# ChaoqinRobotics/LINS---LiDAR-inertial-SLAM

Measured on NVIDIA H100. Metric: ESKF iterations/sec, higher is better.
Workload: dtype f64 (f32 association)

## Files before the change

lins---lidar-inertial-slam_b200/csrc/cuda/lins_assoc_az.cuh:

```cuda
#pragma once
#include "lins_kernels.cuh"

namespace lins_dev {

struct AzIndex {
  const float4* pts;
  const aztab_t* bstart;
  const int (*elev)[2];
  int nb, nrings, T;
};
__device__ __forceinline__ int float_key(float f) { const int i = __float_as_int(f); return i >= 0 ? i : i ^ 0x7fffffff; }
__device__ __forceinline__ float key_float(int k) { return __int_as_float(k >= 0 ? k : k ^ 0x7fffffff); }
__device__ __forceinline__ float slope_of(float x, float y, float z) {
  return __fdiv_rn(z, sqrtf(__fadd_rn(__fmul_rn(x, x), __fmul_rn(y, y))));
}
__device__ __forceinline__ float ring_lower_bound(const AzIndex& ix, int r, float zq, float rq) {
  const float lo = key_float(ix.elev[r][0]), hi = key_float(ix.elev[r][1]);
  const float a = __fmaf_rn(lo, rq, -zq), b = __fmaf_rn(-hi, rq, zq);
  const float m = a > b ? lo : hi;
  const float bound = fmaxf(a, b) * rsqrtf(__fmaf_rn(m, m, 1.f)) * 0.998f - 1.0e-4f;
  return hi - lo < 1.0e30f ? bound : -1.f;
}

__device__ __forceinline__ int az_bin(float x, float y, int nb) {
  const float a = atan2f(y, x);
  int b = (int)floorf((a + kPiF) * ((float)nb * (0.5f / kPiF)));
  return min(max(b, 0), nb - 1);
}
__device__ __forceinline__ int az_bins_for(int nrings, int tab) {
  int p2 = 1;
  while (p2 < nrings) p2 <<= 1;
  return tab / p2;
}

__device__ __forceinline__ int cnt16_add1(unsigned* cnt, int b) {
  const int sh = (b & 1) * 16;
  return (int)((atomicAdd(&cnt[b >> 1], 1u << sh) >> sh) & 0xffffu);
}
template <int TAB>
__device__ void az_build(const float4* __restrict__ src, int T, float4* dst, aztab_t* table, unsigned* cnt, int* scan_tmp, int nb, int (*elev)[2]) {
  unsigned short* cnt16 = reinterpret_cast<unsigned short*>(cnt);
  for (int w = threadIdx.x; w <= TAB / 2; w += kThreads) cnt[w] = 0u;
  for (int r = threadIdx.x; r < kMaxRing; r += kThreads) { elev[r][0] = float_key(3.0e38f); elev[r][1] = float_key(-3.0e38f); }
  __syncthreads();
  for (int j = threadIdx.x; j < T; j += kThreads) {
    const float4 t = __ldg(&src[j]);
    cnt16_add1(cnt, (int)t.w * nb + az_bin(t.x, t.y, nb));
    const float e = slope_of(t.x, t.y, t.z);
    if (fabsf(e) < 1.0e30f) { const int k = float_key(e); atomicMin(&elev[(int)t.w][0], k); atomicMax(&elev[(int)t.w][1], k); }
    else { atomicMin(&elev[(int)t.w][0], float_key(-3.0e38f)); atomicMax(&elev[(int)t.w][1], float_key(3.0e38f)); }
  }
  __syncthreads();
  constexpr int PER = TAB / kThreads;
  static_assert(PER >= 1 && PER * kThreads == TAB, "table size must be a multiple of the block size");
  int loc[PER];
  int sum = 0;
#pragma unroll
  for (int k = 0; k < PER; ++k) { loc[k] = cnt16[threadIdx.x * PER + k]; sum += loc[k]; }
  scan_tmp[threadIdx.x] = sum;
  __syncthreads();
  if (threadIdx.x < 32) {
    constexpr int PW = kThreads / 32;
    int part[PW];
    int s = 0;
#pragma unroll
    for (int k = 0; k < PW; ++k) { part[k] = scan_tmp[threadIdx.x * PW + k]; s += part[k]; }
    int incl = s;
#pragma unroll
    for (int m = 1; m < 32; m <<= 1) { const int o = __shfl_up_sync(0xffffffffu, incl, m); if ((int)threadIdx.x >= m) incl += o; }
    int run = incl - s;
#pragma unroll
    for (int k = 0; k < PW; ++k) { const int v = part[k]; scan_tmp[threadIdx.x * PW + k] = run; run += v; }
    if (threadIdx.x == 31) table[TAB] = (aztab_t)incl;
  }
  __syncthreads();
  {
    int run = scan_tmp[threadIdx.x];
#pragma unroll
    for (int k = 0; k < PER; ++k) { cnt16[threadIdx.x * PER + k] = (unsigned short)run; table[threadIdx.x * PER + k] = (aztab_t)run; run += loc[k]; }
  }
  __syncthreads();
  for (int j = threadIdx.x; j < T; j += kThreads) {
    const float4 t = __ldg(&src[j]);
    const int pos = cnt16_add1(cnt, (int)t.w * nb + az_bin(t.x, t.y, nb));
    dst[pos] = make_float4(t.x, t.y, t.z, __int_as_float(((int)t.w << 24) | j));
  }
  __syncthreads();
}

__device__ __forceinline__ float az_halfwidth(float U, float rho) {
  const float r = sqrtf(U) * 1.002f + 1.0e-5f;
  if (!(r < rho)) return 4.0f;
  return asinf(r / rho) + 1.0e-5f;
}
__device__ __forceinline__ void az_window(int nb, float aq, float th, int& blo, int& nbins) {
  const float inv_binw = (float)nb * (0.5f / kPiF);
  nbins = (int)(2.0f * th * inv_binw) + 3;
  if (!(th < kPiF) || nbins >= nb) { blo = 0; nbins = nb; return; }
  int b = (int)floorf((aq - th + kPiF) * inv_binw) - 1;
  b %= nb;
  if (b < 0) b += nb;
  blo = b;
}

__device__ __forceinline__ int slot_index(float w) { return __float_as_int(w) & 0x00ffffff; }
__device__ __forceinline__ int slot_ring(float w) { return (int)((unsigned)__float_as_int(w) >> 24); }
__device__ __forceinline__ int pack_window(int blo, int nbins) { return (blo << 16) | nbins; }
constexpr float kCertMargin = 0.1f;
__device__ __forceinline__ float widen(float U) { const float r = sqrtf(U) + kCertMargin; return r * r; }
__device__ __forceinline__ float rejected_slack(unsigned best_bits, float Bout, float gate) {
  const float db = best_bits >= 0x7f800000u ? Bout : fminf(sqrtf(__uint_as_float(best_bits)), Bout);
  return db - gate * 1.00001f;
}

__device__ __forceinline__ void az_polar(const float4 s, float4& qa) {
  qa.x = atan2f(s.y, s.x);
  qa.y = sqrtf(__fadd_rn(__fmul_rn(s.x, s.x), __fmul_rn(s.y, s.y)));
}
__device__ __forceinline__ int az_nn_window(const AzIndex& ix, float U1, float4& qa) {
  const float Uw = widen(U1);
  int blo, nbins;
  az_window(ix.nb, qa.x, az_halfwidth(Uw, qa.y), blo, nbins);
  qa.w = nbins >= ix.nb ? 3.0e38f : sqrtf(Uw);
  return pack_window(blo, nbins);
}
__device__ __forceinline__ float az_seed_bound(const AzIndex& ix, const float4 s, int seed_slot, float U1) {
  if (seed_slot >= 0 && seed_slot < ix.T) {
    const float4 t = ix.pts[seed_slot];
    const float d = sqdist_f32(s.x, s.y, s.z, t.x, t.y, t.z);
    if (d < U1) U1 = d;
  }
  return U1;
}
__device__ __forceinline__ int az_bin_of_angle(float a, int nb) {
  const int b = (int)floorf((a + kPiF) * ((float)nb * (0.5f / kPiF)));
  return min(max(b, 0), nb - 1);
}
__device__ __forceinline__ float az_bucket_bound(const AzIndex& ix, const float4 s, float az, int ring_guess, float U1) {
  const int bq = az_bin_of_angle(az, ix.nb);
  const int r0 = min(max(ring_guess, 0), ix.nrings - 1);
#pragma unroll 1
  for (int k = 0; k < 3; ++k) {
    const int r = k == 0 ? r0 : (k == 1 ? r0 - 1 : r0 + 1);
    if (k == 1 && U1 < 1.0f) break;
    if (r < 0 || r >= ix.nrings) continue;
    const int base = r * ix.nb;
    int p = ix.bstart[base + max(bq - 1, 0)];
    const int pe = min((int)ix.bstart[base + min(bq + 2, ix.nb)], p + 4);
    for (; p < pe; ++p) U1 = az_seed_bound(ix, s, p, U1);
  }
  return U1;
}
__device__ __forceinline__ int az_prepare_nn(const AzIndex& ix, const float4 s, float nearf, int seed_slot, int ring_guess, float4& qa) {
  qa = make_float4(0.f, 0.f, -1.f, 0.f);
  if (!(s.x == s.x && s.y == s.y && s.z == s.z) || ix.T <= 0) return -1;
  az_polar(s, qa);
  float U1 = az_seed_bound(ix, s, seed_slot, nearf);
  if (seed_slot < 0) U1 = az_bucket_bound(ix, s, qa.x, ring_guess, U1);
  return az_nn_window(ix, U1, qa);
}
constexpr float kProbeSq = 0.25f;
__device__ __forceinline__ int az_probe_window(const AzIndex& ix, const float4 qa, int full_window) {
  int blo, nbins;
  az_window(ix.nb, qa.x, az_halfwidth(kProbeSq, qa.y), blo, nbins);
  return (full_window & 0xffff) > 2 * nbins + 4 ? pack_window(blo, nbins) : -1;
}

struct Top3 {
  unsigned long long k1, k2;
  int p1, p2;
// ... 326 lines not shown
```

lins---lidar-inertial-slam_b200/csrc/cuda/lins_gpu.cu:

```cuda
#include <cuda_runtime.h>

#include <algorithm>
#include <cstddef>
#include <cstdio>
#include <cstdlib>
#include <cstring>
#include <new>
#include <utility>

#include "lins_assoc.cuh"
#include "lins_ctx.hpp"
#include "lins_icp_step.cuh"

using namespace lins_dev;
using namespace lins_capi;

extern "C" int lins_jacobian_parts(int n_units, int sm_count);
extern "C" int lins_launch_jacobian_mma(const lins_dev::BatchView* bv, const lins_dev::KParams* kp, int n_units, int sm_count, int P, double* part_acc,
                                        int* part_cnt, cudaStream_t stream);

namespace {

template <int MODE>
__device__ void unit_prologue(CtaMem& cta, Smem& sm, const BatchView& bv, const KParams& kp, const PassBuffers& pb, int slot) {
  const int tid = threadIdx.x, warp = tid >> 5;
  const int scan = sm.scan;
  if (tid < 20) { const double v = tid < 19 ? bv.state_in[(size_t)scan * 20 + tid] : 0.0; sm.prior[tid] = v; sm.lin[tid] = v; }
  for (int e = tid; e < 108; e += kThreads) {
    const int a = e / 6, c = e % 6;
    sm.Pc[e] = bv.cov_in[(size_t)scan * 324 + col6(c) * 18 + a];
  }
  if (tid == 32) {
    sm.flags[0] = sm.flags[1] = sm.flags[2] = sm.flags[3] = 0; sm.residualNorm = 1e6;
    sm.cnt[0] = sm.cnt[1] = 0;
    sm.iter = MODE == MODE_IESKF ? 0 : kp.iter0;
    sm.fresh = 0; sm.finished = 0; sm.first_pass = 1; sm.pos_valid = 0; sm.pos_is_slot = 0;
    sm.run = 1;
    if (MODE == MODE_IESKF && kp.num_iter <= 0) { sm.run = 0; sm.finished = 1; cta.any_finished = 1; }
    sm.qs0 = bv.qs_off[scan]; sm.ns = bv.qs_off[scan + 1] - sm.qs0;
    sm.qc0 = bv.qc_off[scan]; sm.nc = bv.qc_off[scan + 1] - sm.qc0;
    sm.ts0 = bv.ts_off[scan]; sm.Ts = bv.ts_off[scan + 1] - sm.ts0;
    sm.tc0 = bv.tc_off[scan]; sm.Tc = bv.tc_off[scan + 1] - sm.tc0;
  }
  __syncthreads();
  check_ring_sorted(bv.ts + sm.ts0, sm.Ts, &sm.sortedS);
  check_ring_sorted(bv.tc + sm.tc0, sm.Tc, &sm.sortedC);
  if (tid == 0) {
    const bool ok = sm.sortedS && sm.sortedC && !nn_separate(bv, scan) && sm.Ts < 65536 && sm.Tc < 65536;
    sm.az_ok = ok ? 1 : 0;
    sm.nringsS = ok && sm.Ts > 0 ? (int)bv.ts[sm.ts0 + sm.Ts - 1].w + 1 : 0;
    sm.nringsC = ok && sm.Tc > 0 ? (int)bv.tc[sm.tc0 + sm.Tc - 1].w + 1 : 0;
    sm.nbS = az_bins_for(sm.nringsS, kAzTabS);
    sm.nbC = az_bins_for(sm.nringsC, kAzTabC);
  }
  __syncthreads();
  if (sm.az_ok) {
    az_build<kAzTabS>(bv.ts + sm.ts0, sm.Ts, bv.az_s + sm.ts0, sm.azTabS, cta.u.build_tab, cta.scan_tmp, sm.nbS, sm.elevS);
    az_build<kAzTabC>(bv.tc + sm.tc0, sm.Tc, bv.az_c + sm.tc0, sm.azTabC, cta.u.build_tab, cta.scan_tmp, sm.nbC, sm.elevC);
  }
  float4* qdst = pb.qpt + (size_t)slot * bv.qtile;
  if (bv.qscratch == nullptr) {
    const uint32_t bytes = (uint32_t)(sm.ns + sm.nc) * 16u;
    if (bytes > 0) {
      if (tid == 0) {
        fence_proxy_async();
        mbar_expect_tx(&cta.mbar, bytes);
        if (sm.ns > 0) tma_load_1d(qdst, bv.qs + sm.qs0, (uint32_t)sm.ns * 16u, &cta.mbar);
        if (sm.nc > 0) tma_load_1d(qdst + sm.ns, bv.qc + sm.qc0, (uint32_t)sm.nc * 16u, &cta.mbar);
      }
      const unsigned int ph = cta.phase;
      mbar_wait(&cta.mbar, ph & 1u);
      __syncthreads();
      if (tid == 0) cta.phase = ph + 1u;
    }
  } else {
    for (int i = tid; i < sm.ns + sm.nc; i += kThreads) qdst[i] = i < sm.ns ? __ldg(bv.qs + sm.qs0 + i) : __ldg(bv.qc + sm.qc0 + i - sm.ns);
  }
  if (warp == 0) iter_consts_warp0(sm);
  __syncthreads();
}

__device__ void unit_tail(CtaMem& cta, Smem& sm, const BatchView& bv, const KParams& kp, const PassBuffers& pb, int slot, double sig2) {
  const int lane = threadIdx.x & 31;
  const int iter = sm.iter;
  lins_report* rep = bv.reports ? bv.reports + sm.scan : nullptr;
  const int nq = sm.ns + sm.nc;
  finish_acc_warp0(sm, pb.wacc + (size_t)slot * pb.nvw * kNAcc, pb.wcnt + (size_t)slot * pb.nvw * 2, (nq + 31) >> 5);
  build_A6_warp0(sm);
  if (slot == 0) LINS_TICK(18);
  if (lane < 6) {
    double y = sm.y6[lane];
    for (int c = 0; c < 6; ++c) y += sm.A6[lane * 6 + c] * sm.dvec[col6(c)];
    sm.X6[lane] = y;
  }
  form_M6(sm, sig2, lane, 32);
  __syncwarp();
  const bool ok = warp_lu_cols<6>(sm.M6, sm.X6, 1);
  __syncwarp();
  if (slot == 0) LINS_TICK(19);
  double u = 0.0;
  if (lane < 18) {
    double kx = 0;
    for (int c = 0; c < 6; ++c) kx += sm.Pc[lane * 6 + c] * sm.X6[c];
    u = ok ? (-kx + sm.dvec[lane]) : __longlong_as_double(0x7ff8000000000000ll);
  }
  const bool hasNaN = __ballot_sync(0xffffffffu, u != u) != 0u;
  if (u != u) u = 0.0;
  if (lane < 18) sm.upd[lane] = u;
  __syncwarp();
  double nrm = 0.0;
  if (lane == 0) for (int a = 0; a < 18; ++a) nrm += sm.upd[a] * sm.upd[a];
  if (lane == 1) nrm = sm.acc[27];
  nrm = sqrt(nrm);
  const double un = __shfl_sync(0xffffffffu, nrm, 0), rnorm = __shfl_sync(0xffffffffu, nrm, 1);
  if (slot == 0) LINS_TICK(21);
  if (lane == 0) {
    if (rep) {
      rep->m_surf[iter] = sm.cnt[0]; rep->m_corner[iter] = sm.cnt[1];
      rep->residual_norm[iter] = rnorm; rep->update_norm[iter] = un;
    }
    if (hasNaN) {
      sm.flags[2] = 1; sm.flags[1] = 1; sm.flags[3] = 1;
    } else if (rnorm > sm.residualNorm * 10) {
      sm.flags[1] = 1; sm.flags[3] = 1;
    } else {
      box_plus(sm);
      if (un <= 1e-2 && !kp.force_all_iters) { sm.flags[0] = 1; sm.flags[3] = 1; }
      sm.residualNorm = rnorm;
    }
    const bool search = (iter % kp.icp_freq) == 0;
    if (search) sm.pos_is_slot = sm.az_ok; else if (!sm.pos_valid) sm.pos_is_slot = 0;
    sm.pos_valid = 1;
    sm.first_pass = 0;
    sm.iter = iter + 1;
    if (sm.flags[3] || iter + 1 >= kp.num_iter) { sm.finished = 1; sm.run = 0; cta.any_finished = 1; }
  }
  __syncwarp();
  if (slot == 0) LINS_TICK(23);
  if (!sm.finished) iter_consts_warp0(sm);
  if (slot == 0) LINS_TICK(25);
}

__device__ void unit_exit(CtaMem& cta, Smem& sm, const BatchView& bv, double sig2) {
  const int tid = threadIdx.x, warp = tid >> 5, lane = tid & 31;
  const int scan = sm.scan, iters = sm.iter;
  const bool diverged = sm.flags[1] != 0;
  auto& ex = cta.u.ex;
  if (!diverged && iters > 0) {
    for (int e = tid; e < 324; e += kThreads) {
      const int r = e / 18, c = e % 18;
      ex.P[e] = bv.cov_in[(size_t)scan * 324 + c * 18 + r];
    }
    form_M6(sm, sig2, tid, kThreads);
    for (int e = tid; e < 72; e += kThreads) {
      const int a = e / 12, c = e % 12;
      ex.X6[e] = c < 6 ? sm.A6[a * 6 + c] : (a == c - 6 ? 1.0 : 0.0);
    }
    __syncthreads();
    if (warp == 0) {
      const bool ok = warp_lu_cols<6>(sm.M6, ex.X6, 12);
      if (!ok) for (int e = lane; e < 72; e += 32) ex.X6[e] = __longlong_as_double(0x7ff8000000000000ll);
// ... 25 lines not shown
  for (int e = tid; e < 324; e += kThreads) {
    const int r = e / 18, c = e % 18;
    double v;
    if (diverged || iters == 0) v = bv.cov_in[(size_t)scan * 324 + c * 18 + r];
    else v = 0.5 * (ex.P[r * 18 + c] + ex.P[c * 18 + r]);
    bv.cov_out[(size_t)scan * 324 + c * 18 + r] = v;
  }
  if (tid == 0) {
    lins_scan_result& o = bv.results[scan];
    o.scan_id = scan;
    o.iters = (uint16_t)iters;
    o.flags = (uint16_t)((sm.flags[0] ? 1 : 0) | (sm.flags[1] ? 2 : 0) | (sm.flags[2] ? 4 : 0));
    const double* st = diverged ? sm.prior : sm.lin;
    o.pose[0] = st[0]; o.pose[1] = st[1]; o.pose[2] = st[2];
    o.pose[3] = st[6]; o.pose[4] = st[7]; o.pose[5] = st[8]; o.pose[6] = st[9];
    lins_report* rep = bv.reports ? bv.reports + scan : nullptr;
    if (rep) { rep->iters = iters; rep->converged = sm.flags[0]; rep->diverged = sm.flags[1]; rep->has_nan = sm.flags[2]; }
  }
  __syncthreads();
}

template <int MODE>
__global__ void __launch_bounds__(kThreads, kMinCtas) lins_ieskf_kernel(const __grid_constant__ BatchView bv,
                                                                     const __grid_constant__ KParams kp) {
  extern __shared__ __align__(128) unsigned char smem_raw[];
  const int S = bv.nslots;
  PassBuffers pb;
  const PassLayout lay = pass_layout(S, bv.qtile, &pb, smem_raw, bv.qscratch, blockIdx.x, bv.qscratch_stride);
  CtaMem& cta = *reinterpret_cast<CtaMem*>(smem_raw);
  Smem* slots = reinterpret_cast<Smem*>(smem_raw + lay.slots);
  const int tid = threadIdx.x, warp = tid >> 5;
  const double sig2 = kp.lidar_std * kp.lidar_std;

  if (tid == 0) {
    mbar_init(&cta.mbar, 1);
    cta.phase = 0;
    cta.wl_n[0] = 0; cta.wl_n[1] = 0; cta.wl_tn[0] = 0; cta.wl_tn[1] = 0; cta.wl_thead[0] = 0; cta.wl_thead[1] = 0; cta.wl_head[0] = 0; cta.wl_head[1] = 0; cta.dbg[0] = 0; cta.dbg[1] = 0;
    cta.exhausted = 0; cta.any_finished = 0;
    for (int s = 0; s < S; ++s) { slots[s].scan = -1; slots[s].fresh = 0; slots[s].run = 0; slots[s].finished = 0; }
    fence_mbar_init();
    cta.tlast = clock64();
  }
  __syncthreads();
  const long long t_cta0 = clock64();

  for (;;) {
    if (tid == 0) {
      int nact = 0, nfresh = 0;
      for (int s = 0; s < S; ++s) {
        Smem& sm = slots[s];
        if (MODE == MODE_ICP_REDUCE) {
          while (sm.scan < 0 && !cta.exhausted) {
            const int u = atomicAdd(bv.work_counter, 1);
            if (u >= bv.n_scans) cta.exhausted = 1;
            else if (!bv.icp_done || !bv.icp_done[(size_t)u * kIcpDoneStride]) { sm.scan = u; sm.fresh = 1; }
          }
        } else if (sm.scan < 0 && !cta.exhausted) {
          const int u = atomicAdd(bv.work_counter, 1);
          if (u < bv.n_scans) { sm.scan = u; sm.fresh = 1; } else cta.exhausted = 1;
        }
        if (sm.scan >= 0) ++nact;
        if (sm.fresh) ++nfresh;
      }
      cta.n_active = nact; cta.any_fresh = nfresh;
      cta.pass_first = 0;
      if (bv.timers) {
        int nrun = 0;
        for (int s = 0; s < S; ++s) { if (slots[s].fresh || (slots[s].run && slots[s].first_pass)) cta.pass_first = 1; if (slots[s].scan >= 0) ++nrun; }
        atomicAdd((unsigned long long*)&bv.timers[cta.pass_first ? 62 : 30], 1ull);
        atomicAdd((unsigned long long*)&bv.timers[cta.pass_first ? 63 : 31], (unsigned long long)nrun);
      }
    }
    __syncthreads();
    if (cta.n_active == 0) {
      if (bv.timers && tid == 0) {
        const unsigned long long busy = (unsigned long long)(clock64() - t_cta0);
        atomicAdd((unsigned long long*)&bv.timers[26], busy);
        atomicMax((unsigned long long*)&bv.timers[27], busy);
      }
      break;
    }
    LINS_TICK(1);
    if (cta.any_fresh) {
      for (int s = 0; s < S; ++s)
        if (slots[s].fresh) unit_prologue<MODE>(cta, slots[s], bv, kp, pb, s);
      if (tid == 0) {
        int leg = 0, idx = 0;
        for (int s = 0; s < S; ++s) if (slots[s].scan >= 0) { if (slots[s].az_ok) idx = 1; else leg = 1; }
        cta.any_legacy = leg; cta.any_indexed = idx;
      }
      __syncthreads();
      LINS_TICK(0);
    }

    association_pass<MODE>(cta, slots, bv, kp, pb);
    if (MODE == MODE_IESKF) {
      if (warp < S && slots[warp].run) unit_tail(cta, slots[warp], bv, kp, pb, warp, sig2);
    } else {
      if (warp < S && slots[warp].run) {
        Smem& sm = slots[warp];
        const int lane = tid & 31;
        const int scan = sm.scan;
        finish_acc_warp0(sm, pb.wacc + (size_t)warp * pb.nvw * kNAcc, pb.wcnt + (size_t)warp * pb.nvw * 2, (sm.ns + sm.nc + 31) >> 5);
        if (bv.accum) {
          if (lane < kNAcc) bv.accum[(size_t)scan * 32 + lane] = sm.acc[lane];
          if (lane == 28) bv.accum[(size_t)scan * 32 + 28] = (double)sm.cnt[0];
          if (lane == 29) bv.accum[(size_t)scan * 32 + 29] = (double)sm.cnt[1];
        }
        __syncwarp();
        if (lane == 0) { sm.scan = -1; sm.run = 0; }
      }
    }
    __syncthreads();
    LINS_TICK(8);
    if (MODE == MODE_IESKF && cta.any_finished) {
      for (int s = 0; s < S; ++s) {
        if (!slots[s].finished) continue;
        unit_exit(cta, slots[s], bv, sig2);
        if (tid == 0) { slots[s].scan = -1; slots[s].finished = 0; slots[s].run = 0; }
      }
      if (tid == 0) cta.any_finished = 0;
      __syncthreads();
      LINS_TICK(9);
    }
  }
}


__device__ __forceinline__ void to_end_consts(const double* __restrict__ lin, double* sphi, double* srn, double* sq) {
  if (threadIdx.x == 0) {
    q4 q; q.x = lin[6]; q.y = lin[7]; q.z = lin[8]; q.w = lin[9];
    d3 phi = Quat2axis(q);
    sphi[0] = phi.x; sphi[1] = phi.y; sphi[2] = phi.z;
    srn[0] = lin[0]; srn[1] = lin[1]; srn[2] = lin[2];
    sq[0] = q.x; sq[1] = q.y; sq[2] = q.z; sq[3] = q.w;
  }
  __syncthreads();
}
__device__ __forceinline__ float4 to_end_point(float4 p, const double* sphi, const double* srn, const double* sq, double scan_period) {
  float fi = p.w - (float)((int)p.w);
  double s = (1.f / scan_period) * fi;
  q4 r = axis2Quat(mk3(s * sphi[0], s * sphi[1], s * sphi[2]));
  d3 P1 = add3(qrot(r, mk3(p.x, p.y, p.z)), mk3(s * srn[0], s * srn[1], s * srn[2]));
  q4 q; q.x = sq[0]; q.y = sq[1]; q.z = sq[2]; q.w = sq[3];
  d3 P2 = qrot(qinverse(q), sub3(P1, mk3(srn[0], srn[1], srn[2])));
  p.x = (float)P2.x; p.y = (float)P2.y; p.z = (float)P2.z;
  return p;
}

__global__ void lins_transform_to_end_csr_kernel(float4* __restrict__ pts, const int* __restrict__ off, const double* __restrict__ lin,
                                                 const unsigned char* __restrict__ run, double scan_period) {
  __shared__ double sphi[3], srn[3], sq[4];
  const int u = blockIdx.x;
  if (!run[u]) return;
  to_end_consts(lin + (size_t)u * 20, sphi, srn, sq);
  for (int i = off[u] + threadIdx.x; i < off[u + 1]; i += blockDim.x) pts[i] = to_end_point(pts[i], sphi, srn, sq, scan_period);
}

__global__ void lins_transform_to_end_kernel(float4* __restrict__ pts, int n, const double* __restrict__ lin,
                                             double scan_period, lins_point* __restrict__ out32) {
  __shared__ double sphi[3], srn[3], sq[4];
  to_end_consts(lin, sphi, srn, sq);
  int i = blockIdx.x * blockDim.x + threadIdx.x;
  if (i >= n) return;
  float4 p = to_end_point(pts[i], sphi, srn, sq, scan_period);
  pts[i] = p;
  if (out32) {
    float4* o = reinterpret_cast<float4*>(out32 + i);
    o[0] = make_float4(p.x, p.y, p.z, 1.0f);
    o[1] = make_float4(p.w, 0.f, 0.f, 0.f);
  }
}

KParams make_kparams(const lins_params& p, int mode, int iter0) {
// ... 499 lines not shown
```

lins---lidar-inertial-slam_b200/csrc/cuda/lins_kernels.cuh:

```cuda
#pragma once
#include "../../../include/lins_gpu.h"
#include "lins_device_math.cuh"

namespace lins_dev {

constexpr int kThreads = 512;
constexpr int kMinCtas = 1;
constexpr int kWarps = kThreads / 32;
constexpr int kMaxSlots = 4;
constexpr int kMaxRing = 128;
constexpr int kNAcc = 28;
constexpr int kNNChunk = 1024;
constexpr int kAzTabS = 4096;
constexpr int kAzTabC = 1024;
constexpr float kPiF = 3.14159265358979f;
constexpr unsigned long long kKeyMax = 0xFFFFFFFFFFFFFFFFull;

enum KernelMode { MODE_IESKF = 0, MODE_ASSOC = 1, MODE_ICP_REDUCE = 2, MODE_JACOBIAN = 3 };

struct BatchView {
  int n_scans;
  const float4* qs; const int* qs_off;
  const float4* qc; const int* qc_off;
  const float4* ts; const int* ts_off;
// ... 1 lines not shown
  const float4* nn_s; const int* nn_s_off;
  const float4* nn_c; const int* nn_c_off;
  const unsigned char* nn_stale;
  const double* state_in;
  const double* cov_in;
  double* state_out;
  double* cov_out;
  lins_scan_result* results;
  lins_report* reports;
  int* ind_s;
  int* ind_c;
  float* sel_s; float* sel_c;
  float* coeff_s; float* coeff_c;
  unsigned char* mask_s; unsigned char* mask_c;
  double* accum;
  float4* az_s; float4* az_c;
  int* work_counter;
  long long* timers;
  int qtile;
  int nslots;
  const int* icp_done;
  unsigned char* qscratch;
  size_t qscratch_stride;
};

struct IcpState {
  double matP[36];
  int iters, converged, done, pad;
};
constexpr int kIcpDoneStride = (int)(sizeof(IcpState) / sizeof(int));
static_assert(sizeof(IcpState) % sizeof(int) == 0, "IcpState stride");

struct KParams {
  int num_iter, icp_freq, force_all_iters, mode, iter0;
  double nearest_sq, lidar_std, lidar_scale, scan_period;
};

__device__ __forceinline__ bool nn_separate(const BatchView& bv, int scan) {
  return bv.nn_s != nullptr && (bv.nn_stale == nullptr || bv.nn_stale[scan] != 0);
}

__device__ __forceinline__ unsigned long long pack_key(float d, unsigned int lo) {
  return ((unsigned long long)__float_as_uint(d) << 32) | lo;
}
__device__ __forceinline__ unsigned long long shfl_xor_u64(unsigned long long v, int m) {
  return __shfl_xor_sync(0xffffffffu, v, m);
}
__device__ __forceinline__ unsigned long long warp_min_u64(unsigned long long v) {
#pragma unroll
  for (int m = 16; m > 0; m >>= 1) {
    unsigned long long o = shfl_xor_u64(v, m);
    v = o < v ? o : v;
  }
  return v;
}

typedef unsigned short aztab_t;

struct alignas(16) Smem {
  double prior[20];
  double Pc[18 * 6];
  double lin[20];
  double phi[3];
  double R[9];
  double Rinv[9];
  double dvec[18];
  double acc[kNAcc + 4];
  double A6[36];
  double y6[6];
  double M6[36];
  double X6[6];
  double upd[18];
  double residualNorm;
  int flags[4];
  int cnt[2];
  int scan;
  int iter;
  int fresh;
  int run;
  int finished;
  int first_pass;
  int pos_valid, pos_is_slot;
  int qs0, ns, qc0, nc, ts0, Ts, tc0, Tc;
  int sortedS, sortedC;
  int az_ok;
  int nbS, nbC, nringsS, nringsC;
  aztab_t azTabS[kAzTabS + 2];
  aztab_t azTabC[kAzTabC + 2];
  int elevS[kMaxRing][2], elevC[kMaxRing][2];
};

struct CtaMem {
  union {
    unsigned build_tab[kAzTabS / 2 + 1];
    struct { double P[324], X[324], U[108], V[108], X6[72]; } ex;
    double fold[kWarps][64];
  } u;
  int scan_tmp[kThreads];
  int wl_n[2], wl_head[2];
  int wl_tn[2], wl_thead[2];
  int dbg[2];
  int n_active, any_fresh, any_finished, any_legacy, any_indexed, exhausted, pass_first;
  unsigned long long mbar;
  unsigned int phase;
  long long tlast;
};
static_assert(sizeof(((CtaMem*)nullptr)->u.fold) <= sizeof(((CtaMem*)nullptr)->u.build_tab), "the fold stage must not grow the CTA");

#define LINS_TICK(k)                                                                   \
  do {                                                                                 \
    if (bv.timers && threadIdx.x == 0) {                                               \
      const long long _t = clock64();                                                  \
      atomicAdd((unsigned long long*)&bv.timers[k], (unsigned long long)(_t - cta.tlast)); \
      cta.tlast = _t;                                                                   \
    }                                                                                  \
  } while (0)
#define LINS_TICK_PASS(k) LINS_TICK((k) + (cta.pass_first ? 32 : 0))

__device__ __forceinline__ float4 transform_to_start(const float4 p, const Smem& sm, double scan_period) {
  float fi = p.w - (float)((int)p.w);
  double s = (1.f / scan_period) * fi;
  d3 v = mk3(s * sm.phi[0], s * sm.phi[1], s * sm.phi[2]);
  q4 r = axis2Quat(v);
  d3 P2 = mk3((double)p.x, (double)p.y, (double)p.z);
  d3 rp = qrot(r, P2);
  d3 t = mk3(s * sm.lin[0], s * sm.lin[1], s * sm.lin[2]);
  float4 o;
  o.x = (float)(rp.x + t.x); o.y = (float)(rp.y + t.y); o.z = (float)(rp.z + t.z); o.w = p.w;
  return o;
}

__device__ inline void check_ring_sorted(const float4* __restrict__ tgt, int T, int* sorted_flag) {
  if (threadIdx.x == 0) *sorted_flag = 1;
  __syncthreads();
  for (int j = threadIdx.x; j < T; j += kThreads) {
    const int rj = (int)__ldg(&tgt[j]).w;
    const int rp = j > 0 ? (int)__ldg(&tgt[j - 1]).w : -1;
    if (rj < 0 || rj >= kMaxRing || (j > 0 && rj < rp)) *sorted_flag = 0;
  }
  __syncthreads();
}

__device__ inline void nn_brute(const float4* sel, unsigned long long* key, int nq, const float4* __restrict__ tgt, int T) {
  const int warp = threadIdx.x >> 5, lane = threadIdx.x & 31;
  const int nqg = (nq + 31) >> 5, nch = (T + kNNChunk - 1) / kNNChunk;
  for (int item = warp; item < nqg * nch; item += kWarps) {
    const int qg = item % nqg, ch = item / nqg;
    const int qi = qg * 32 + lane;
    const bool valid = qi < nq;
    const float4 s = valid ? sel[qi] : make_float4(0.f, 0.f, 0.f, 0.f);
    const int j0 = ch * kNNChunk, j1 = min(T, j0 + kNNChunk);
    float best = __int_as_float(0x7f800000);
    int bi = -1;
#pragma unroll 4
    for (int j = j0; j < j1; ++j) {
      const float4 t = __ldg(&tgt[j]);
      const float d = sqdist_f32(s.x, s.y, s.z, t.x, t.y, t.z);
      if (d < best) { best = d; bi = j; }
    }
    if (valid && bi >= 0) atomicMin(&key[qi], pack_key(best, (unsigned)bi));
  }
}


__device__ __forceinline__ unsigned int order_fwd(int j) { return (unsigned)j; }
__device__ __forceinline__ unsigned int order_bwd(int j) { return 0x80000000u | (unsigned)(0x7fffffff - j); }
__device__ __forceinline__ int order_decode(unsigned int o) { return (o & 0x80000000u) ? (0x7fffffff - (int)(o & 0x7fffffffu)) : (int)o; }

template <bool SURF>
__device__ void walk_seq(const float4 s, int c, const float4* __restrict__ tgt, int T, int fwdBound, float nearf,
                         int& i2, int& i3) {
  const int cr = (int)__ldg(&tgt[c]).w;
  float m2 = nearf, m3 = nearf;
  i2 = -1; i3 = -1;
  for (int j = c + 1; j < fwdBound; ++j) {
    const float4 t = __ldg(&tgt[j]);
    const int rj = (int)t.w;
    if ((double)rj > (double)cr + 2.5) break;
    const float d = sqdist_f32(t.x, t.y, t.z, s.x, s.y, s.z);
    if (SURF) {
      if (rj <= cr) { if (d < m2) { m2 = d; i2 = j; } }
      else { if (d < m3) { m3 = d; i3 = j; } }
    } else {
      if (rj > cr) { if (d < m2) { m2 = d; i2 = j; } }
    }
  }
  for (int j = c - 1; j >= 0; --j) {
    const float4 t = __ldg(&tgt[j]);
    const int rj = (int)t.w;
    if ((double)rj < (double)cr - 2.5) break;
    const float d = sqdist_f32(t.x, t.y, t.z, s.x, s.y, s.z);
    if (SURF) {
      if (rj >= cr) { if (d < m2) { m2 = d; i2 = j; } }
      else { if (d < m3) { m3 = d; i3 = j; } }
    } else {
      if (rj < cr) { if (d < m2) { m2 = d; i2 = j; } }
    }
  }
}

__device__ __forceinline__ bool plane_residual(const float4 sel, const float4 t1, const float4 t2, const float4 t3,
                                               bool weighted, float4& coeff) {
  d3 P0 = mk3(sel.x, sel.y, sel.z), P1 = mk3(t1.x, t1.y, t1.z), P2 = mk3(t2.x, t2.y, t2.z), P3 = mk3(t3.x, t3.y, t3.z);
  d3 M = cross3(sub3(P1, P2), sub3(P1, P3));
  double r = dot3(sub3(P0, P1), M);
  double m = norm3(M);
  float res = (float)(r / m);
  d3 jac = div3(M, m);
  float s = 1.f;
  if (weighted) {
    float n2 = __fadd_rn(__fadd_rn(__fmul_rn(sel.x, sel.x), __fmul_rn(sel.y, sel.y)), __fmul_rn(sel.z, sel.z));
    float rt = sqrtf(sqrtf(n2));
    s = (float)(1.0 - 1.8 * (double)fabsf(res) / (double)rt);
  }
  if ((double)s > 0.1 && res != 0.f) {
    coeff.x = (float)((double)s * jac.x); coeff.y = (float)((double)s * jac.y); coeff.z = (float)((double)s * jac.z);
    coeff.w = __fmul_rn(s, res);
    return true;
  }
  return false;
}
__device__ __forceinline__ bool line_residual(const float4 sel, const float4 t1, const float4 t2, bool weighted,
                                              float4& coeff) {
// ... 248 lines not shown
```

Before: 7.304 million.

## Batch fresh-slot prologues and fuse azimuth index build into fewer barriers

Replaces the per-slot prologue with a single pass over all fresh slots. It counts directly into each slot's table and folds the ring-sortedness check into the counting loop. The scan becomes a reduce-then-scan over warp sums, and the scatter walks the prefix ends downward with atomicSub. The query TMA load now overlaps with index construction, and the loads are batched per thread. These steps cut the number of __syncthreads and global passes per fresh scan, but they interleave slot work and drop the scratch build table, which adds complexity and a risk around edge cases such as a table-count overflow.

```diff
diff --git a/lins---lidar-inertial-slam_b200/csrc/cuda/lins_assoc_az.cuh b/lins---lidar-inertial-slam_b200/csrc/cuda/lins_assoc_az.cuh
--- a/lins---lidar-inertial-slam_b200/csrc/cuda/lins_assoc_az.cuh
+++ b/lins---lidar-inertial-slam_b200/csrc/cuda/lins_assoc_az.cuh
@@ -33,59 +33,87 @@
   return tab / p2;
 }
 
-__device__ __forceinline__ int cnt16_add1(unsigned* cnt, int b) {
+constexpr int kBuildBatch = 4;
+__device__ __forceinline__ void cnt16_add1(unsigned* cnt, int b) { atomicAdd(&cnt[b >> 1], 1u << ((b & 1) * 16)); }
+__device__ __forceinline__ int cnt16_sub1(unsigned* cnt, int b) {
   const int sh = (b & 1) * 16;
-  return (int)((atomicAdd(&cnt[b >> 1], 1u << sh) >> sh) & 0xffffu);
+  return (int)((atomicSub(&cnt[b >> 1], 1u << sh) >> sh) & 0xffffu) - 1;
 }
 template <int TAB>
-__device__ void az_build(const float4* __restrict__ src, int T, float4* dst, aztab_t* table, unsigned* cnt, int* scan_tmp, int nb, int (*elev)[2]) {
-  unsigned short* cnt16 = reinterpret_cast<unsigned short*>(cnt);
-  for (int w = threadIdx.x; w <= TAB / 2; w += kThreads) cnt[w] = 0u;
+__device__ __forceinline__ void az_clear(aztab_t* table, int (*elev)[2]) {
+  unsigned* w = reinterpret_cast<unsigned*>(table);
+  for (int k = threadIdx.x; k < TAB / 2 + 1; k += kThreads) w[k] = 0u;
   for (int r = threadIdx.x; r < kMaxRing; r += kThreads) { elev[r][0] = float_key(3.0e38f); elev[r][1] = float_key(-3.0e38f); }
-  __syncthreads();
-  for (int j = threadIdx.x; j < T; j += kThreads) {
-    const float4 t = __ldg(&src[j]);
-    cnt16_add1(cnt, (int)t.w * nb + az_bin(t.x, t.y, nb));
-    const float e = slope_of(t.x, t.y, t.z);
-    if (fabsf(e) < 1.0e30f) { const int k = float_key(e); atomicMin(&elev[(int)t.w][0], k); atomicMax(&elev[(int)t.w][1], k); }
-    else { atomicMin(&elev[(int)t.w][0], float_key(-3.0e38f)); atomicMax(&elev[(int)t.w][1], float_key(3.0e38f)); }
-  }
-  __syncthreads();
+}
+__device__ __forceinline__ void az_count(const float4* __restrict__ src, int T, int nrings, int nb, aztab_t* table, int (*elev)[2], int* ok) {
+  unsigned* cnt = reinterpret_cast<unsigned*>(table);
+  bool bad = false;
+  for (int j0 = 0; j0 < T; j0 += kBuildBatch * kThreads) {
+    float4 t[kBuildBatch];
+    float wp[kBuildBatch];
+#pragma unroll
+    for (int k = 0; k < kBuildBatch; ++k) {
+      const int j = j0 + k * kThreads + (int)threadIdx.x;
+      t[k] = j < T ? __ldg(&src[j]) : make_float4(0.f, 0.f, 0.f, 0.f);
+      wp[k] = j > 0 && j < T ? __ldg(&src[j - 1].w) : -1.f;
+    }
+#pragma unroll
+    for (int k = 0; k < kBuildBatch; ++k) {
+      if (j0 + k * kThreads + (int)threadIdx.x >= T) break;
+      const int r = (int)t[k].w;
+      if (r < 0 || r >= nrings || r < (int)wp[k]) { bad = true; continue; }
+      cnt16_add1(cnt, r * nb + az_bin(t[k].x, t[k].y, nb));
+      const float e = slope_of(t[k].x, t[k].y, t[k].z);
+      if (fabsf(e) < 1.0e30f) { const int key = float_key(e); atomicMin(&elev[r][0], key); atomicMax(&elev[r][1], key); }
+      else { atomicMin(&elev[r][0], float_key(-3.0e38f)); atomicMax(&elev[r][1], float_key(3.0e38f)); }
+    }
+  }
+  if (bad) *ok = 0;
+}
+template <int TAB>
+__device__ __forceinline__ void az_scan_sums(const aztab_t* table, int* wsum) {
   constexpr int PER = TAB / kThreads;
   static_assert(PER >= 1 && PER * kThreads == TAB, "table size must be a multiple of the block size");
+  int sum = 0;
+#pragma unroll
+  for (int k = 0; k < PER; ++k) sum += table[threadIdx.x * PER + k];
+  const int tot = __reduce_add_sync(0xffffffffu, sum);
+  if ((threadIdx.x & 31) == 0) wsum[threadIdx.x >> 5] = tot;
+}
+template <int TAB>
+__device__ __forceinline__ void az_scan_ends(aztab_t* table, const int* wsum) {
+  constexpr int PER = TAB / kThreads;
+  const int lane = threadIdx.x & 31, warp = threadIdx.x >> 5;
   int loc[PER];
   int sum = 0;
 #pragma unroll
-  for (int k = 0; k < PER; ++k) { loc[k] = cnt16[threadIdx.x * PER + k]; sum += loc[k]; }
-  scan_tmp[threadIdx.x] = sum;
-  __syncthreads();
-  if (threadIdx.x < 32) {
-    constexpr int PW = kThreads / 32;
-    int part[PW];
-    int s = 0;
-#pragma unroll
-    for (int k = 0; k < PW; ++k) { part[k] = scan_tmp[threadIdx.x * PW + k]; s += part[k]; }
-    int incl = s;
-#pragma unroll
-    for (int m = 1; m < 32; m <<= 1) { const int o = __shfl_up_sync(0xffffffffu, incl, m); if ((int)threadIdx.x >= m) incl += o; }
-    int run = incl - s;
-#pragma unroll
-    for (int k = 0; k < PW; ++k) { const int v = part[k]; scan_tmp[threadIdx.x * PW + k] = run; run += v; }
-    if (threadIdx.x == 31) table[TAB] = (aztab_t)incl;
-  }
-  __syncthreads();
-  {
-    int run = scan_tmp[threadIdx.x];
-#pragma unroll
-    for (int k = 0; k < PER; ++k) { cnt16[threadIdx.x * PER + k] = (unsigned short)run; table[threadIdx.x * PER + k] = (aztab_t)run; run += loc[k]; }
-  }
-  __syncthreads();
-  for (int j = threadIdx.x; j < T; j += kThreads) {
-    const float4 t = __ldg(&src[j]);
-    const int pos = cnt16_add1(cnt, (int)t.w * nb + az_bin(t.x, t.y, nb));
-    dst[pos] = make_float4(t.x, t.y, t.z, __int_as_float(((int)t.w << 24) | j));
-  }
-  __syncthreads();
+  for (int k = 0; k < PER; ++k) { loc[k] = table[threadIdx.x * PER + k]; sum += loc[k]; }
+  int incl = sum;
+#pragma unroll
+  for (int m = 1; m < 32; m <<= 1) { const int o = __shfl_up_sync(0xffffffffu, incl, m); if (lane >= m) incl += o; }
+  int run = incl - sum;
+  for (int w = 0; w < warp; ++w) run += wsum[w];
+#pragma unroll
+  for (int k = 0; k < PER; ++k) { run += loc[k]; table[threadIdx.x * PER + k] = (aztab_t)run; }
+  if (threadIdx.x == kThreads - 1) table[TAB] = (aztab_t)run;
+}
+__device__ __forceinline__ void az_scatter(const float4* __restrict__ src, int T, int nb, float4* dst, aztab_t* table) {
+  unsigned* cnt = reinterpret_cast<unsigned*>(table);
+  for (int j0 = 0; j0 < T; j0 += kBuildBatch * kThreads) {
+    float4 t[kBuildBatch];
+#pragma unroll
+    for (int k = 0; k < kBuildBatch; ++k) {
+      const int j = j0 + k * kThreads + (int)threadIdx.x;
+      t[k] = j < T ? __ldg(&src[j]) : make_float4(0.f, 0.f, 0.f, 0.f);
+    }
+#pragma unroll
+    for (int k = 0; k < kBuildBatch; ++k) {
+      const int j = j0 + k * kThreads + (int)threadIdx.x;
+      if (j >= T) break;
+      const int pos = cnt16_sub1(cnt, (int)t[k].w * nb + az_bin(t[k].x, t[k].y, nb));
+      dst[pos] =make_float4(t[k].x, t[k].y, t[k].z, __int_as_float(((int)t[k].w << 24) | j));
+    }
+  }
 }
 
 __device__ __forceinline__ float az_halfwidth(float U, float rho) {
diff --git a/lins---lidar-inertial-slam_b200/csrc/cuda/lins_gpu.cu b/lins---lidar-inertial-slam_b200/csrc/cuda/lins_gpu.cu
--- a/lins---lidar-inertial-slam_b200/csrc/cuda/lins_gpu.cu
+++ b/lins---lidar-inertial-slam_b200/csrc/cuda/lins_gpu.cu
@@ -22,61 +22,112 @@
 namespace {
 
 template <int MODE>
-__device__ void unit_prologue(CtaMem& cta, Smem& sm, const BatchView& bv, const KParams& kp, const PassBuffers& pb, int slot) {
+__device__ void fresh_prologues(CtaMem& cta, Smem* slots, const BatchView& bv, const KParams& kp, const PassBuffers& pb) {
   const int tid = threadIdx.x, warp = tid >> 5;
-  const int scan = sm.scan;
-  if (tid < 20) { const double v = tid < 19 ? bv.state_in[(size_t)scan * 20 + tid] : 0.0; sm.prior[tid] = v; sm.lin[tid] = v; }
-  for (int e = tid; e < 108; e += kThreads) {
-    const int a = e / 6, c = e % 6;
-    sm.Pc[e] = bv.cov_in[(size_t)scan * 324 + col6(c) * 18 + a];
-  }
-  if (tid == 32) {
-    sm.flags[0] = sm.flags[1] = sm.flags[2] = sm.flags[3] = 0; sm.residualNorm = 1e6;
-    sm.cnt[0] = sm.cnt[1] = 0;
-    sm.iter = MODE == MODE_IESKF ? 0 : kp.iter0;
-    sm.fresh = 0; sm.finished = 0; sm.first_pass = 1; sm.pos_valid = 0; sm.pos_is_slot = 0;
-    sm.run = 1;
-    if (MODE == MODE_IESKF && kp.num_iter <= 0) { sm.run = 0; sm.finished = 1; cta.any_finished = 1; }
-    sm.qs0 = bv.qs_off[scan]; sm.ns = bv.qs_off[scan + 1] - sm.qs0;
-    sm.qc0 = bv.qc_off[scan]; sm.nc = bv.qc_off[scan + 1] - sm.qc0;
-    sm.ts0 = bv.ts_off[scan]; sm.Ts = bv.ts_off[scan + 1] - sm.ts0;
-    sm.tc0 = bv.tc_off[scan]; sm.Tc = bv.tc_off[scan + 1] - sm.tc0;
+  const int S = bv.nslots;
+  for (int s = 0; s < S; ++s) {
+    Smem& sm = slots[s];
+    if (!sm.fresh) continue;
+    const int scan = sm.scan;
+    if (tid < 20) { const double v = tid < 19 ? bv.state_in[(size_t)scan * 20 + tid] : 0.0; sm.prior[tid] = v; sm.lin[tid] = v; }
+    for (int e = tid; e < 108; e += kThreads) {
+      const int a = e / 6, c = e % 6;
+      sm.Pc[e] = bv.cov_in[(size_t)scan * 324 + col6(c) * 18 + a];
+    }
+    if (tid == 32 * (s + 1)) {
+      sm.flags[0] = sm.flags[1] = sm.flags[2] = sm.flags[3] = 0; sm.residualNorm = 1e6;
+      sm.cnt[0] = sm.cnt[1] = 0;
+      sm.iter = MODE == MODE_IESKF ? 0 : kp.iter0;
+      sm.finished = 0; sm.first_pass = 1; sm.pos_valid = 0; sm.pos_is_slot = 0;
+      sm.run = 1;
+      if (MODE == MODE_IESKF && kp.num_iter <= 0) { sm.run = 0; sm.finished = 1; cta.any_finished = 1; }
+      sm.qs0 = bv.qs_off[scan]; sm.ns = bv.qs_off[scan + 1] - sm.qs0;
+      sm.qc0 = bv.qc_off[scan]; sm.nc = bv.qc_off[scan + 1] - sm.qc0;
+      sm.ts0 = bv.ts_off[scan]; sm.Ts = bv.ts_off[scan + 1] - sm.ts0;
+      sm.tc0 = bv.tc_off[scan]; sm.Tc = bv.tc_off[scan + 1] - sm.tc0;
+      const bool fit = !nn_separate(bv, scan) && sm.Ts < 65536 && sm.Tc < 65536;
+      const int rS = fit && sm.Ts > 0 ? (int)bv.ts[sm.ts0 + sm.Ts - 1].w : -1;
+      const int rC = fit && sm.Tc > 0 ? (int)bv.tc[sm.tc0 + sm.Tc - 1].w : -1;
+      const bool ok = fit && (sm.Ts == 0 || rS >= 0) && (sm.Tc == 0 || rC >= 0) && rS < kMaxRing && rC < kMaxRing;
+      sm.az_ok = ok ? 1 : 0;
+      sm.nringsS = ok ? rS + 1 : 0;
+      sm.nringsC = ok ? rC + 1 : 0;
+      sm.nbS = az_bins_for(sm.nringsS, kAzTabS);
+      sm.nbC = az_bins_for(sm.nringsC, kAzTabC);
+    }
+    az_clear<kAzTabS>(sm.azTabS, sm.elevS);
+    az_clear<kAzTabC>(sm.azTabC, sm.elevC);
   }
   __syncthreads();
-  check_ring_sorted(bv.ts + sm.ts0, sm.Ts, &sm.sortedS);
-  check_ring_sorted(bv.tc + sm.tc0, sm.Tc, &sm.sortedC);
-  if (tid == 0) {
-    const bool ok = sm.sortedS && sm.sortedC && !nn_separate(bv, scan) && sm.Ts < 65536 && sm.Tc < 65536;
-    sm.az_ok = ok ? 1 : 0;
-    sm.nringsS = ok && sm.Ts > 0 ? (int)bv.ts[sm.ts0 + sm.Ts - 1].w + 1 : 0;
-    sm.nringsC = ok && sm.Tc > 0 ? (int)bv.tc[sm.tc0 + sm.Tc - 1].w + 1 : 0;
-    sm.nbS = az_bins_for(sm.nringsS, kAzTabS);
-    sm.nbC = az_bins_for(sm.nringsC, kAzTabC);
-  }
-  __syncthreads();
-  if (sm.az_ok) {
-    az_build<kAzTabS>(bv.ts + sm.ts0, sm.Ts, bv.az_s + sm.ts0, sm.azTabS, cta.u.build_tab, cta.scan_tmp, sm.nbS, sm.elevS);
-    az_build<kAzTabC>(bv.tc + sm.tc0, sm.Tc, bv.az_c + sm.tc0, sm.azTabC, cta.u.build_tab, cta.scan_tmp, sm.nbC, sm.elevC);
-  }
-  float4* qdst = pb.qpt + (size_t)slot * bv.qtile;
+  uint32_t qbytes = 0;
+  for (int s = 0; s < S; ++s) if (slots[s].fresh) qbytes += (uint32_t)(slots[s].ns + slots[s].nc) * 16u;
   if (bv.qscratch == nullptr) {
-    const uint32_t bytes = (uint32_t)(sm.ns + sm.nc) * 16u;
-    if (bytes > 0) {
-      if (tid == 0) {
-        fence_proxy_async();
-        mbar_expect_tx(&cta.mbar, bytes);
+    if (tid == 0 && qbytes > 0) {
+      fence_proxy_async();
+      mbar_expect_tx(&cta.mbar, qbytes);
+      for (int s = 0; s < S; ++s) {
+        const Smem& sm = slots[s];
+        if (!sm.fresh) continue;
+        float4* qdst = pb.qpt + (size_t)s * bv.qtile;
         if (sm.ns > 0) tma_load_1d(qdst, bv.qs + sm.qs0, (uint32_t)sm.ns * 16u, &cta.mbar);
         if (sm.nc > 0) tma_load_1d(qdst + sm.ns, bv.qc + sm.qc0, (uint32_t)sm.nc * 16u, &cta.mbar);
       }
-      const unsigned int ph = cta.phase;
-      mbar_wait(&cta.mbar, ph & 1u);
-      __syncthreads();
-      if (tid == 0) cta.phase = ph + 1u;
     }
   } else {
-    for (int i = tid; i < sm.ns + sm.nc; i += kThreads) qdst[i] = i < sm.ns ? __ldg(bv.qs + sm.qs0 + i) : __ldg(bv.qc + sm.qc0 + i - sm.ns);
-  }
-  if (warp == 0) iter_consts_warp0(sm);
+    for (int s = 0; s < S; ++s) {
+      const Smem& sm = slots[s];
+      if (!sm.fresh) continue;
+      float4* qdst = pb.qpt + (size_t)s * bv.qtile;
+      for (int i = tid; i < sm.ns + sm.nc; i += kThreads) qdst[i] = i < sm.ns ? __ldg(bv.qs + sm.qs0 + i) : __ldg(bv.qc + sm.qc0 + i - sm.ns);
+    }
+  }
+  for (int s = 0; s < S; ++s) {
+    Smem& sm = slots[s];
+    if (!sm.fresh || (sm.nringsS == 0 && sm.nringsC == 0)) continue;
+#pragma unroll 1
+    for (int c = 0; c < 2; ++c)
+      az_count(c ? bv.tc + sm.tc0 : bv.ts + sm.ts0, c ? sm.Tc : sm.Ts, c ? sm.nringsC : sm.nringsS, c ? sm.nbC : sm.nbS,
+               c ? sm.azTabC : sm.azTabS, c ? sm.elevC : sm.elevS, &sm.az_ok);
+  }
+  __syncthreads();
+  for (int s = 0; s < S; ++s) {
+    Smem& sm = slots[s];
+    if (!sm.fresh) continue;
+    if (!sm.az_ok) {
+      if (tid == 32 * (s + 1)) { sm.nringsS = 0; sm.nringsC = 0; sm.nbS = az_bins_for(0, kAzTabS); sm.nbC = az_bins_for(0, kAzTabC); }
+      continue;
+    }
+    az_scan_sums<kAzTabS>(sm.azTabS, cta.wsum[2 * s]);
+    az_scan_sums<kAzTabC>(sm.azTabC, cta.wsum[2 * s + 1]);
+  }
+  __syncthreads();
+  for (int s = 0; s < S; ++s) {
+    Smem& sm = slots[s];
+    if (!sm.fresh || !sm.az_ok) continue;
+    az_scan_ends<kAzTabS>(sm.azTabS, cta.wsum[2 * s]);
+    az_scan_ends<kAzTabC>(sm.azTabC, cta.wsum[2 * s + 1]);
+  }
+  __syncthreads();
+  for (int s = 0; s < S; ++s) {
+    Smem& sm = slots[s];
+    if (!sm.fresh || !sm.az_ok) continue;
+#pragma unroll 1
+    for (int c = 0; c < 2; ++c)
+      az_scatter(c ? bv.tc + sm.tc0 : bv.ts + sm.ts0, c ? sm.Tc : sm.Ts, c ? sm.nbC : sm.nbS, c ? bv.az_c + sm.tc0 : bv.az_s + sm.ts0,
+                 c ? sm.azTabC : sm.azTabS);
+  }
+  if (bv.qscratch == nullptr && qbytes > 0) mbar_wait(&cta.mbar, cta.phase & 1u);
+  __syncthreads();
+  if (warp < S && slots[warp].fresh) {
+    iter_consts_warp0(slots[warp]);
+    if ((tid & 31) == 0) slots[warp].fresh = 0;
+  }
+  if (tid == 0) {
+    if (bv.qscratch == nullptr && qbytes > 0) cta.phase += 1u;
+    int leg = 0, idx = 0;
+    for (int s = 0; s < S; ++s) if (slots[s].scan >= 0) { if (slots[s].az_ok) idx = 1; else leg = 1; }
+    cta.any_legacy = leg; cta.any_indexed = idx;
+  }
   __syncthreads();
 }
 
@@ -268,14 +319,7 @@
     }
     LINS_TICK(1);
     if (cta.any_fresh) {
-      for (int s = 0; s < S; ++s)
-        if (slots[s].fresh) unit_prologue<MODE>(cta, slots[s], bv, kp, pb, s);
-      if (tid == 0) {
-        int leg = 0, idx = 0;
-        for (int s = 0; s < S; ++s) if (slots[s].scan >= 0) { if (slots[s].az_ok) idx = 1; else leg = 1; }
-        cta.any_legacy = leg; cta.any_indexed = idx;
-      }
-      __syncthreads();
+      fresh_prologues<MODE>(cta, slots, bv, kp, pb);
       LINS_TICK(0);
     }
 
diff --git a/lins---lidar-inertial-slam_b200/csrc/cuda/lins_kernels.cuh b/lins---lidar-inertial-slam_b200/csrc/cuda/lins_kernels.cuh
--- a/lins---lidar-inertial-slam_b200/csrc/cuda/lins_kernels.cuh
+++ b/lins---lidar-inertial-slam_b200/csrc/cuda/lins_kernels.cuh
@@ -107,21 +107,19 @@
   int first_pass;
   int pos_valid, pos_is_slot;
   int qs0, ns, qc0, nc, ts0, Ts, tc0, Tc;
-  int sortedS, sortedC;
   int az_ok;
   int nbS, nbC, nringsS, nringsC;
-  aztab_t azTabS[kAzTabS + 2];
-  aztab_t azTabC[kAzTabC + 2];
+  alignas(4) aztab_t azTabS[kAzTabS + 2];
+  alignas(4) aztab_t azTabC[kAzTabC + 2];
   int elevS[kMaxRing][2], elevC[kMaxRing][2];
 };
 
 struct CtaMem {
   union {
-    unsigned build_tab[kAzTabS / 2 + 1];
     struct { double P[324], X[324], U[108], V[108], X6[72]; } ex;
     double fold[kWarps][64];
   } u;
-  int scan_tmp[kThreads];
+  int wsum[2 * kMaxSlots][kWarps];
   int wl_n[2], wl_head[2];
   int wl_tn[2], wl_thead[2];
   int dbg[2];
@@ -130,7 +128,6 @@
   unsigned int phase;
   long long tlast;
 };
-static_assert(sizeof(((CtaMem*)nullptr)->u.fold) <= sizeof(((CtaMem*)nullptr)->u.build_tab), "the fold stage must not grow the CTA");
 
 #define LINS_TICK(k)                                                                   \
   do {                                                                                 \
@@ -153,17 +150,6 @@
   float4 o;
   o.x = (float)(rp.x + t.x); o.y = (float)(rp.y + t.y); o.z = (float)(rp.z + t.z); o.w = p.w;
   return o;
-}
-
-__device__ inline void check_ring_sorted(const float4* __restrict__ tgt, int T, int* sorted_flag) {
-  if (threadIdx.x == 0) *sorted_flag = 1;
-  __syncthreads();
-  for (int j = threadIdx.x; j < T; j += kThreads) {
-    const int rj = (int)__ldg(&tgt[j]).w;
-    const int rp = j > 0 ? (int)__ldg(&tgt[j - 1]).w : -1;
-    if (rj < 0 || rj >= kMaxRing || (j > 0 && rj < rp)) *sorted_flag = 0;
-  }
-  __syncthreads();
 }
 
 __device__ inline void nn_brute(const float4* sel, unsigned long long* key, int nq, const float4* __restrict__ tgt, int T) {
```

New measurement: 7.373 million (median of 6 runs). Within noise of the previous version (+0.9%).
